# caishiqing/voice-tts

Measured on AMD Instinct MI355X. Metric: audio_seconds_per_second, higher is better.
Workload: dtype bf16

## Files before the change

include/ixtts_hip.h:

```cpp
#ifndef IXTTS_HIP_H
#define IXTTS_HIP_H

#include <stddef.h>
#include <stdint.h>

#ifdef __cplusplus
extern "C" {
#endif

#define IXTTS_OK 0
#define IXTTS_ERR_ARG (-1)
#define IXTTS_ERR_HIP (-2)
#define IXTTS_ERR_STATE (-3)
#define IXTTS_ERR_NOMEM (-4)
#define IXTTS_ERR_NAME (-5)

const char* ixtts_version(void);
const char* ixtts_last_error(void);

int ixtts_aa_snake_f32(const float* x_dev, float* y_dev, const float* up12_dev, const float* down12_dev,
                       const float* log_alpha_dev, const float* log_beta_dev, int B, int C, int T, void* stream);

size_t ixtts_attn_full_workspace_bytes(int B, int H, int T);
int ixtts_attn_full_f32(const float* q_dev, const float* k_dev, const float* v_dev, float* out_dev, int B, int H, int T,
// ... 144 lines not shown
int ixtts_gpt_decode(ixtts_gpt* h, int n_active, int n_steps, const ixtts_sampler_cfg* sc, void* stream);
int ixtts_gpt_decode_slots(ixtts_gpt* h, int n_active, int n_steps, const ixtts_sampler_cfg* per_slot, const uint32_t* rng_stream,
                           void* stream);
int ixtts_gpt_read(ixtts_gpt* h, int b, int32_t* ids_host, int cap, int* n_ids, int* finished, void* stream);
int ixtts_gpt_read_logits(ixtts_gpt* h, int b, float* logits_host, void* stream);
int ixtts_gpt_read_probs(ixtts_gpt* h, int b, float* probs_host, void* stream);
int ixtts_gpt_set_bans(ixtts_gpt* h, int slot, const int32_t* always_host, int n_always, const int32_t* first_host, int n_first,
                       void* stream);
int ixtts_gpt_set_sequence_bias(ixtts_gpt* h, int slot, const int32_t* ids_flat_host, const int32_t* lens_host, const float* biases_host,
                                int n, void* stream);
int ixtts_gpt_set_forced_eos(ixtts_gpt* h, int slot, const int32_t* ids_host, int n, void* stream);
int ixtts_gpt_force_next(ixtts_gpt* h, int b, int32_t token, void* stream);

int ixtts_gpt_beam_begin(ixtts_gpt* h, int num_beams, void* stream);
int ixtts_gpt_beam_decode(ixtts_gpt* h, int n_steps, const ixtts_sampler_cfg* sc, void* stream);
int ixtts_gpt_beam_read(ixtts_gpt* h, int max_new, int32_t* ids_host, int cap, int* n_ids, int* done, float* score,
                        float* beam_scores_host, int32_t* last_tokens_host, int32_t* beam_idx_host, void* stream);
int ixtts_gpt_beam_force(ixtts_gpt* h, const int32_t* picks_host, int n, void* stream);

int ixtts_gpt_beam_begin_group(ixtts_gpt* h, int group, int num_beams, uint64_t rng_stream, void* stream);
int ixtts_gpt_beam_park_group(ixtts_gpt* h, int group, void* stream);
int ixtts_gpt_beam_decode_groups(ixtts_gpt* h, int n_groups, int n_steps, const ixtts_sampler_cfg* sc, void* stream);
int ixtts_gpt_beam_decode_groups_cfg(ixtts_gpt* h, int n_groups, int n_steps, const ixtts_sampler_cfg* per_group, void* stream);
int ixtts_gpt_beam_read_group(ixtts_gpt* h, int group, int max_new, int32_t* ids_host, int cap, int* n_ids, int* done, float* score,
                              float* beam_scores_host, int32_t* last_tokens_host, int32_t* beam_idx_host, void* stream);
int ixtts_gpt_beam_force_group(ixtts_gpt* h, int group, const int32_t* picks_host, int n, void* stream);

int ixtts_gpt_latent(ixtts_gpt* h, const float* prefix_dev, int n_prefix, const int32_t* codes_dev, int n,
                     float* latent_dev, void* stream);
int ixtts_gpt_latent_many(ixtts_gpt* h, int n, const float* const* prefix_dev, const int* n_prefix, const int32_t* const* codes_dev,
                          const int* n_codes, float* const* latent_dev, int rows_max, void* stream);
int ixtts_gpt_latent_plan(const int* n_prefix, const int* n_codes, int n, int row_cap, int* pass_of);

int ixtts_gpt_bench_gemv(ixtts_gpt* h, int which, int layer, int batch, void* stream);
double ixtts_gpt_step_bytes(const ixtts_gpt* h, int B, int S);

int ixtts_gpt_max_batch(void);
int ixtts_gpt_max_batch_for(int weight_dtype);

int ixtts_gpt_destroy(ixtts_gpt* h);

#define IXTTS_QWEN_TOPK_MAX 64
#define IXTTS_QWEN_MAX_EOS 8
#define IXTTS_QWEN_MAX_SLOTS 4

typedef struct ixtts_qwen_cfg {
  int hidden_size;
  int layers;
  int heads;
  int kv_heads;
  int head_dim;
  int intermediate_size;
  int vocab_size;
  float rms_norm_eps;
  float rope_theta;
  int tie_word_embeddings;
  int max_seq;
  int weight_dtype;
  int n_eos;
  int eos_ids[IXTTS_QWEN_MAX_EOS];
} ixtts_qwen_cfg;

typedef struct ixtts_qwen_sampling {
  int do_sample;
  float temperature;
  int top_k;
// ... 60 lines not shown
```

voice-tts_amd/_lib.py:

```python
import ctypes as C
import os

HERE = os.path.dirname(os.path.abspath(__file__))
LIB_PATH = os.environ.get("IXTTS_LIB") or os.path.join(HERE, "libixtts_hip.so")

MAX_STAGES = 8
MAX_RESK = 4
BIGVGAN_TILE_SLOTS = 6


class BigVGANCfg(C.Structure):
    _fields_ = [
        ("num_mels", C.c_int), ("upsample_initial_channel", C.c_int), ("n_stages", C.c_int),
        ("upsample_rates", C.c_int * MAX_STAGES), ("upsample_kernel_sizes", C.c_int * MAX_STAGES),
        ("n_resblock_kernels", C.c_int), ("resblock_kernel_sizes", C.c_int * MAX_RESK),
        ("resblock_dilations", (C.c_int * 3) * MAX_RESK), ("max_frames", C.c_int), ("fast_sin", C.c_int),
    ]


class GptCfg(C.Structure):
    _fields_ = [
        ("model_dim", C.c_int), ("layers", C.c_int), ("heads", C.c_int), ("n_mel_codes", C.c_int),
        ("n_mel_pos", C.c_int), ("n_text_tokens", C.c_int), ("n_text_pos", C.c_int),
        ("start_mel_token", C.c_int), ("stop_mel_token", C.c_int), ("max_seq", C.c_int),
# ... 91 lines not shown
    "ixtts_bigvgan_forward_varlen": (C.c_int, [_P, _P, _P, _P, C.c_int, C.c_int, _P, _P]),
    "ixtts_bigvgan_tile_launches": (C.c_int, [_P, C.POINTER(C.c_int64), C.POINTER(C.c_int)]),
    "ixtts_bigvgan_flops": (C.c_double, [_P, C.c_int, C.c_int]),
    "ixtts_bigvgan_destroy": (C.c_int, [_P]),
    "ixtts_gpt_create": (C.c_int, [C.POINTER(_P), C.POINTER(GptCfg)]),
    "ixtts_gpt_set_tensor": (C.c_int, [_P, C.c_char_p, _P, C.POINTER(C.c_int64), C.c_int]),
    "ixtts_gpt_finalize": (C.c_int, [_P]),
    "ixtts_gpt_arena": (C.c_int, [_P, C.POINTER(_P), C.POINTER(C.c_size_t)]),
    "ixtts_gpt_adopt_arena": (C.c_int, [_P]),
    "ixtts_gpt_share_arena": (C.c_int, [_P, _P]),
    "ixtts_gpt_prefill": (C.c_int, [_P, C.c_int, _P, C.c_int, C.c_int, _P]),
    "ixtts_gpt_prefill_many": (C.c_int, [_P, C.c_int, C.POINTER(C.c_int), C.POINTER(_P), C.POINTER(C.c_int), C.POINTER(C.c_int), C.c_int, _P]),
    "ixtts_gpt_prefill_plan": (C.c_int, [C.POINTER(C.c_int), C.POINTER(C.c_int), C.c_int, C.c_int, C.POINTER(C.c_int)]),
    "ixtts_gpt_decode": (C.c_int, [_P, C.c_int, C.c_int, C.POINTER(SamplerCfg), _P]),
    "ixtts_gpt_decode_slots": (C.c_int, [_P, C.c_int, C.c_int, C.POINTER(SamplerCfg), C.POINTER(C.c_uint32), _P]),
    "ixtts_gpt_read": (C.c_int, [_P, C.c_int, _P, C.c_int, C.POINTER(C.c_int), C.POINTER(C.c_int), _P]),
    "ixtts_gpt_read_logits": (C.c_int, [_P, C.c_int, _P, _P]),
    "ixtts_gpt_beam_begin": (C.c_int, [_P, C.c_int, _P]),
    "ixtts_gpt_beam_decode": (C.c_int, [_P, C.c_int, C.POINTER(SamplerCfg), _P]),
    "ixtts_gpt_beam_read": (C.c_int, [_P, C.c_int, _P, C.c_int, C.POINTER(C.c_int), C.POINTER(C.c_int), C.POINTER(C.c_float), _P, _P, _P, _P]),
    "ixtts_gpt_beam_force": (C.c_int, [_P, _P, C.c_int, _P]),
    "ixtts_gpt_beam_begin_group": (C.c_int, [_P, C.c_int, C.c_int, C.c_uint64, _P]),
    "ixtts_gpt_beam_park_group": (C.c_int, [_P, C.c_int, _P]),
    "ixtts_gpt_beam_decode_groups": (C.c_int, [_P, C.c_int, C.c_int, C.POINTER(SamplerCfg), _P]),
    "ixtts_gpt_beam_decode_groups_cfg": (C.c_int, [_P, C.c_int, C.c_int, C.POINTER(SamplerCfg), _P]),
    "ixtts_gpt_beam_read_group":(C.c_int, [_P, C.c_int, C.c_int, _P, C.c_int, C.POINTER(C.c_int), C.POINTER(C.c_int), C.POINTER(C.c_float), _P, _P, _P, _P]),
    "ixtts_gpt_beam_force_group": (C.c_int, [_P, C.c_int, _P, C.c_int, _P]),
    "ixtts_gpt_read_probs": (C.c_int, [_P, C.c_int, _P, _P]),
    "ixtts_gpt_force_next": (C.c_int, [_P, C.c_int, C.c_int32, _P]),
    "ixtts_gpt_set_bans": (C.c_int, [_P, C.c_int, _P, C.c_int, _P, C.c_int, _P]),
    "ixtts_gpt_set_sequence_bias": (C.c_int, [_P, C.c_int, _P, _P, _P, C.c_int, _P]),
    "ixtts_gpt_set_forced_eos": (C.c_int, [_P, C.c_int, _P, C.c_int, _P]),
    "ixtts_gpt_latent": (C.c_int, [_P, _P, C.c_int, _P, C.c_int, _P, _P]),
    "ixtts_gpt_latent_many": (C.c_int, [_P, C.c_int, C.POINTER(_P), C.POINTER(C.c_int), C.POINTER(_P), C.POINTER(C.c_int), C.POINTER(_P), C.c_int, _P]),
    "ixtts_gpt_latent_plan": (C.c_int, [C.POINTER(C.c_int), C.POINTER(C.c_int), C.c_int, C.c_int, C.POINTER(C.c_int)]),
    "ixtts_gpt_bench_gemv": (C.c_int, [_P, C.c_int, C.c_int, C.c_int, _P]),
    "ixtts_gpt_step_bytes": (C.c_double, [_P, C.c_int, C.c_int]),
    "ixtts_gpt_max_batch": (C.c_int, []),
    "ixtts_gpt_max_batch_for": (C.c_int, [C.c_int]),
    "ixtts_gpt_destroy": (C.c_int, [_P]),
    "ixtts_qwen_create": (C.c_int, [C.POINTER(_P), C.POINTER(QwenCfg)]),
    "ixtts_qwen_set_tensor": (C.c_int, [_P, C.c_char_p, _P, C.POINTER(C.c_int64), C.c_int]),
    "ixtts_qwen_finalize": (C.c_int, [_P]),
    "ixtts_qwen_prefill": (C.c_int, [_P, _P, C.c_int, _P]),
    "ixtts_qwen_step": (C.c_int, [_P, C.c_int, C.POINTER(QwenSampling), _P]),
    "ixtts_qwen_read": (C.c_int, [_P, _P, C.c_int, C.POINTER(C.c_int), C.POINTER(C.c_int), _P]),
    "ixtts_qwen_generate": (C.c_int, [_P, C.c_int, C.POINTER(QwenSampling), _P, C.c_int, C.POINTER(C.c_int), C.POINTER(C.c_int), _P]),
    "ixtts_qwen_read_logits": (C.c_int, [_P, _P, _P]),
    "ixtts_qwen_read_kept": (C.c_int, [_P, _P, _P, C.c_int, C.POINTER(C.c_int), _P]),
    "ixtts_qwen_draw": (C.c_int, [_P, C.c_uint64, C.c_int, _P, _P]),
    "ixtts_qwen_step_bytes": (C.c_double, [_P, C.c_int]),
    "ixtts_qwen_create_slots": (C.c_int, [C.POINTER(_P), C.POINTER(QwenCfg), C.c_int]),
    "ixtts_qwen_prefill_slots": (C.c_int, [_P, C.c_int, _P, _P, _P]),
    "ixtts_qwen_step_slots": (C.c_int, [_P, C.c_int, C.c_int, C.POINTER(QwenSampling), _P]),
    "ixtts_qwen_generate_slots": (C.c_int, [_P, C.c_int, C.c_int, C.POINTER(QwenSampling), _P]),
    "ixtts_qwen_read_slot": (C.c_int, [_P, C.c_int, _P, C.c_int, C.POINTER(C.c_int), C.POINTER(C.c_int), _P]),
    "ixtts_qwen_read_logits_slot": (C.c_int, [_P, C.c_int, _P, _P]),
    "ixtts_qwen_read_kept_slot": (C.c_int, [_P, C.c_int, _P, _P, C.c_int, C.POINTER(C.c_int), _P]),
    "ixtts_qwen_destroy": (C.c_int, [_P]),
    "ixtts_resample_tile": (C.c_int, []),
    "ixtts_resample_varlen_f32": (C.c_int, [_P, C.c_long, _P, C.c_long, _P, C.c_int, C.c_long, _P, C.c_long, _P, C.c_int, C.c_int, C.c_int, C.c_int, _P]),
    "ixtts_pcm_assemble": (C.c_int, [_P, C.c_long, _P, C.c_long, _P, C.c_int, C.c_int, _P]),
    "ixtts_loudness_measure": (C.c_int, [_P, C.c_long, _P, C.c_int, _P, _P, C.c_int, C.c_long, _P, _P, C.c_long, _P]),
    "ixtts_loudness_gain": (C.c_int, [_P, _P, C.c_long, _P, _P, C.c_int, _P, _P, _P]),
    "ixtts_pcm_assemble_gain": (C.c_int, [_P, C.c_long, _P, C.c_long, _P, C.c_int, _P, C.c_int, C.c_int, _P]),
}
# ... 57 lines not shown
```

voice-tts_amd/csrc/gpt_engine.h:

```cpp
#pragma once
#include <map>
#include <string>
#include <vector>

#include "common.h"

namespace ixtts {

constexpr int MAXB = 32;
constexpr int MAXB_F32 = 16;
constexpr int MAXB_REG = 4;
constexpr int STEPS_PER_GRAPH = 8;
constexpr int BEAM_MAX = 4;
constexpr int MAXG = MAXB / 2;
constexpr int BEAM_LCP_STRIDE = BEAM_MAX * BEAM_MAX + BEAM_MAX;
constexpr int BEAM_FORCED_STRIDE = 2 * BEAM_MAX;

enum TKind { T_VEC = 0, T_MAT_T = 1, T_MAT_N = 2, T_EMB = 3 };

struct TDesc {
  size_t off = 0;
  int kind = T_VEC;
  int64_t d0 = 0, d1 = 0;
  size_t stage_off = 0;
// ... 57 lines not shown
  unsigned int rng_host[ixtts::MAXB] = {};
  float* scratch = nullptr;
  size_t scratch_floats = 0;
  hipStream_t cap_stream = nullptr;
  hipGraphExec_t step_exec[ixtts::MAXB + 1][ixtts::NBKT + 1] = {};
  hipGraphExec_t multi_exec[ixtts::MAXB + 1][ixtts::NBKT + 1] = {};
  bool mlp_fused = false;
  void* wprx = nullptr;
  float* mlp_part = nullptr;
  unsigned* mlp_ctr = nullptr;
  float* h2 = nullptr;
  float* hc = nullptr;
  bool wide = false;
  int pf_per = 2;
  bool attn_split = true;
  int attn_bucket = ixtts::NBKT;
  int host_prompt_len[ixtts::MAXB + 2];
  int host_gen_est[ixtts::MAXB + 2];
  int num_beams = 0;
  int beam_groups = 1;
  bool group_live[ixtts::MAXG] = {};
  bool group_begun[ixtts::MAXG] = {};
  unsigned long long* beam_stream = nullptr;
  float *beam_scores = nullptr, *hyp_score = nullptr, *hyp_worst = nullptr;
  int *beam_src = nullptr, *hyp_len = nullptr, *n_hyp = nullptr, *beam_done = nullptr, *beam_forced_flag = nullptr;
  int32_t *hyp_tok = nullptr, *beam_forced = nullptr;
  float* beam_cand_v = nullptr;
  int *beam_cand_i = nullptr, *beam_cand_n = nullptr;
  bool beam_every_row = false;
  int* beam_lcp = nullptr;
  hipGraphExec_t beam_exec[ixtts::MAXG + 1][ixtts::NBKT + 1] = {}, beam_multi_exec[ixtts::MAXG + 1][ixtts::NBKT + 1] = {};
  int beam_exec_nb = 0;
  float *rx = nullptr, *rxn = nullptr, *rq = nullptr, *ratt = nullptr, *rff = nullptr;
  std::vector<uint8_t> pf_host;
  uint8_t* pf_dev = nullptr;
  size_t pf_bytes = 0;
  std::vector<uint8_t> lm_host;
  uint8_t* lm_dev = nullptr;
  size_t lm_bytes = 0;
};

#define A_F32(off) reinterpret_cast<float*>(h->arena + (off))
#define A_PTR(off) reinterpret_cast<void*>(h->arena + (off))



namespace ixtts {
int forward_rows(ixtts_gpt* h, int slot, int T, int pos0, int valid_from, hipStream_t st);
}

namespace ixtts {
struct PackSeq {
  const float* embeds;
  int slot, T, pos0, row0;
};
struct PackedPass {
  const PackSeq* seqs;
  const int* tiles;
  const int* row_at;
  const int* row_seq;
  int n_seq, n_tiles, T;
  bool keys_rebased = false;
};
struct LatentSeq {
  const float* prefix;
  const int32_t* codes;
// ... 19 lines not shown
```

voice-tts_amd/csrc/gpt_engine.hip:

```cpp
#define IXTTS_ENGINE_TU 1
#include <type_traits>

#include "gpt_engine.h"
#include "gpt_kernels.h"
#include "gpt_wide.h"

using namespace ixtts;

#ifdef IXTTS_TRACE
static int g_trace_seq = 0;
#define IXTTS_TRACE_ARG , g_trace_seq++
#else
#define IXTTS_TRACE_ARG
#endif
template <typename WT, typename KVT, int K, int ROWS, int UNITS, int B, int INP, int EPI, int WPB = 4, bool XLDS = false>
static int launch_gemv(const GemvArgs& a, hipStream_t st) {
  auto kern = gemv_reg_kernel<WT, K, ROWS, UNITS, B, INP, EPI, KVT, WPB, XLDS>;
  const int n_units = (a.N + ROWS - 1) / ROWS;
  const int grid = ceil_div(n_units, WPB * UNITS);
  hipLaunchKernelGGL(kern, dim3(grid), dim3(64 * WPB), 0, st, a.wt, a.xin, a.bias, a.out, a.N, a.slot0, a.out_stride, a.smax, a.kcache, a.vcache,
                     a.cur_len, a.heads, a.nsplit, a.ln_w, a.ln_b, a.aux, a.xout IXTTS_PF_ARGS(a) IXTTS_TRACE_ARG);
  return IXTTS_OK;
}

// ... 1438 lines not shown
        if (pos + Ti > smax) {
          set_error("gpt_latent_many: entry %d would end at cache position %d of %d", i, pos + Ti, smax);
          return IXTTS_ERR_STATE;
        }
        const int q = tb.n_seq, row0 = tb.rows;
        tb.add(hb, nullptr, slot, Ti, pos, q, row0, h->H * smax);
        ls[q] = LatentSeq{prefix_dev[i], codes_dev[i], latent_dev[i], P, n_codes[i]};
        for (int t = P; t < Ti; ++t) mel_row[mel++] = row0 + t;
        pos += ceil_div(Ti, 64) * 64;
      }
      IX_HIP(hipMemcpyAsync(h->lm_dev, hb, tb.bytes, hipMemcpyHostToDevice, st));
      PackedPass pk = tb.pass(h->lm_dev, 0, n_seq, 0, n_tiles, 0, T);
      pk.keys_rebased = true;
      LatentPass lp;
      lp.lseqs = reinterpret_cast<const LatentSeq*>(h->lm_dev + tb.off_rec);
      lp.mel_row = reinterpret_cast<const int*>(h->lm_dev + tb.off_ints);
      lp.n_mel = n_mel;
      IX_TRY(pack_latent_rows(h, pk, lp, st));
      IX_TRY(forward_rows_packed(h, pk, st));
      IX_TRY(scatter_latent_rows(h, pk, lp, st));
    }
    i0 = i1;
  }
  IX_HIP(hipGetLastError());
  return IXTTS_OK;
}

extern "C" int ixtts_gpt_bench_gemv(ixtts_gpt* h, int which, int layer, int batch, void* stream) {
  NEED_READY(h, "gpt_bench_gemv");
  IX_ARG(layer >= 0 && layer < h->L && batch >= 1 && batch <= h->cfg.max_batch, "gpt_bench_gemv: bad argument");
  return do_gemv_which(h, which, layer, batch, (hipStream_t)stream);
}

extern "C" int ixtts_gpt_max_batch(void) { return MAXB_F32; }

extern "C" int ixtts_gpt_max_batch_for(int weight_dtype) {
  if (weight_dtype == IXTTS_DTYPE_BF16 || weight_dtype == IXTTS_DTYPE_F16) return MAXB;
  return weight_dtype == IXTTS_DTYPE_F32 ? MAXB_F32 : 0;
}

extern "C" double ixtts_gpt_step_bytes(const ixtts_gpt* h, int B, int S) {
  if (!h) return 0.0;
  const double D = h->D, FF = h->FF, V = h->V, L = h->L, es = (double)h->esize;
  double mat = L * (3 * D * D + D * D + 2 * D * FF) + V * D;
  double vec = L * (2 * D + 3 * D + D + 2 * D + FF + D) + 4 * D + V;
  double kv_read = (double)B * 2 * L * S * D * es;
  double kv_write = (double)B * 2 * L * D * es;
  double emb = (double)B * 2 * D * 4;
  return mat * es + vec * 4 + kv_read + kv_write + emb;
}

extern "C" int ixtts_gpt_destroy(ixtts_gpt* h) {
  if (!h) return IXTTS_OK;
  for (int k = 0; k <= NBKT; ++k) {
    for (int b = 0; b <= MAXB; ++b) {
      if (h->step_exec[b][k]) hipGraphExecDestroy(h->step_exec[b][k]);
      if (h->multi_exec[b][k]) hipGraphExecDestroy(h->multi_exec[b][k]);
    }
    for (int g = 0; g <= MAXG; ++g) {
      if (h->beam_exec[g][k]) hipGraphExecDestroy(h->beam_exec[g][k]);
      if (h->beam_multi_exec[g][k]) hipGraphExecDestroy(h->beam_multi_exec[g][k]);
    }
  }
  if (h->cap_stream) hipStreamDestroy(h->cap_stream);
  if (h->arena_borrowed) h->arena = nullptr;
  void* ptrs[] = {h->arena, h->stage, h->kc, h->vc, h->h, h->q, h->ff, h->att, h->part, h->logits, h->rowbuf, h->cur_len, h->gen_count,
// ... 31 lines not shown
```

voice-tts_amd/csrc/gpt_rows.hip:

```cpp
#include "gpt_engine.h"
#include "gpt_kernels.h"

namespace ixtts {

typedef float f32x16 __attribute__((ext_vector_type(16)));
typedef __bf16 bf16x8 __attribute__((ext_vector_type(8)));
typedef _Float16 f16x8 __attribute__((ext_vector_type(8)));

template <typename ET>
struct RowsEl;
template <>
struct RowsEl<bf16> {
  typedef bf16x8 vec8;
  __device__ static __forceinline__ f32x16 mfma(const vec8& a, const vec8& b, const f32x16& c) { return __builtin_amdgcn_mfma_f32_32x32x16_bf16(a, b, c, 0, 0, 0); }
};
template <>
struct RowsEl<f16> {
  typedef f16x8 vec8;
  __device__ static __forceinline__ f32x16 mfma(const vec8& a, const vec8& b, const f32x16& c) { return __builtin_amdgcn_mfma_f32_32x32x16_f16(a, b, c, 0, 0, 0); }
};

__device__ __forceinline__ unsigned int pack_bf16x2(float a, float b) {
  const unsigned short lo = __builtin_bit_cast(unsigned short, (__bf16)a);
  const unsigned short hi = __builtin_bit_cast(unsigned short, (__bf16)b);
// ... 232 lines not shown
          } else {
            const int which = n / g.D;
            const int c = n - which * g.D;
            const int hh = c / HD, d = c % HD;
            KVT* cache = reinterpret_cast<KVT*>(which == 1 ? g.kcache : g.vcache);
            store_kv(cache + ((size_t)hh * g.smax + g.pos0 + m) * HD + d, v);
          }
        }
      }
    }
}

struct GemmArgs16 {
  const unsigned short* A;
  const unsigned short* wt;
  const float* bias;
  void* out;
  void* kcache;
  void* vcache;
  int T, N, K, pos0, smax, D;
};

struct GemmArgs16Packed : GemmArgs16 {
  const int* row_at;
};

__device__ __forceinline__ void glds16(const void* gsrc, void* lds_wave_base) {
  __builtin_amdgcn_global_load_lds((const __attribute__((address_space(1))) void*)gsrc, (__attribute__((address_space(3))) void*)lds_wave_base, 16, 0, 0);
}

constexpr int G16_NBUF = 2;
constexpr int G16_TILE = 128 * 64 * 2;
constexpr int G16_SMEM = G16_NBUF * 2 * G16_TILE;

template <int EPI, typename KVT, typename GA = GemmArgs16>
__global__ __launch_bounds__(256) void gemm_rows_bf16_kernel(GA g) {
  using EL = RowsEl<KVT>;
  typedef typename EL::vec8 vec8;
  constexpr int BM = 128, BN = 128, BK = 64, TILE = G16_TILE, NBUF = G16_NBUF;
  extern __shared__ __attribute__((aligned(1024))) unsigned char smem_raw[];
  unsigned char (*smem)[2][TILE] = reinterpret_cast<unsigned char (*)[2][TILE]>(smem_raw);
  const int tid = threadIdx.x, lane = tid & 63, wave = tid >> 6;
  const int wm = wave >> 1, wn = wave & 1;
  const int l31 = lane & 31, lh = lane >> 5;
  const int m0 = blockIdx.y * BM, n0 = blockIdx.x * BN;

  f32x16 acc[2][2];
#pragma unroll
  for (int mi = 0; mi < 2; ++mi)
#pragma unroll
    for (int j = 0; j < 2; ++j)
#pragma unroll
      for (int r = 0; r < 16; ++r) acc[mi][j][r] = 0.f;

  const unsigned short* asrc[4];
  const unsigned short* wsrc[4];
#pragma unroll
  for (int i = 0; i < 4; ++i) {
    const int row = (wave * 4 + i) * 8 + (lane >> 3);
    const int gran = (lane & 7) ^ ((row >> 1) & 7);
    asrc[i] = g.A + (size_t)min(m0 + row, g.T - 1) * g.K + gran * 8;
    wsrc[i] = g.wt + (size_t)min(n0 + row, g.N - 1) * g.K + gran * 8;
  }
  auto issue = [&](int kt, int buf) {
#pragma unroll
    for (int i = 0; i < 4; ++i) {
      glds16(asrc[i] + kt * BK, &smem[buf][0][(wave * 4 + i) * 1024]);
      glds16(wsrc[i] + kt * BK, &smem[buf][1][(wave * 4 + i) * 1024]);
    }
  };
  const int nkt = g.K / BK;
#pragma unroll
  for (int p = 0; p < NBUF - 1; ++p) issue(min(p, nkt - 1), p);
  for (int kt = 0; kt < nkt; ++kt) {
    issue(min(kt + NBUF - 1, nkt - 1), (kt + NBUF - 1) % NBUF);
    static_assert(NBUF == 2, "the immediate below is 8 * (NBUF - 1)");
    asm volatile("s_waitcnt vmcnt(8)" ::: "memory");
    __builtin_amdgcn_s_barrier();
    const unsigned char* At = smem[kt % NBUF][0];
    const unsigned char* Wt = smem[kt % NBUF][1];
#pragma unroll
    for (int kk = 0; kk < BK / 16; ++kk) {
      vec8 a[2], b[2];
#pragma unroll
      for (int mi = 0; mi < 2; ++mi) {
        const int row = wm * 64 + mi * 32 + l31;
        a[mi] = *reinterpret_cast<const vec8*>(At + row * 128 + (((kk * 2 + lh) ^ ((row >> 1) & 7)) << 4));
      }
#pragma unroll
      for (int j = 0; j < 2; ++j) {
        const int row = wn * 64 + j * 32 + l31;
        b[j] = *reinterpret_cast<const vec8*>(Wt + row * 128 + (((kk * 2 + lh) ^ ((row >> 1) & 7)) << 4));
      }
#pragma unroll
      for (int mi = 0; mi < 2; ++mi)
#pragma unroll
        for (int j = 0; j < 2; ++j) acc[mi][j] = EL::mfma(a[mi], b[j], acc[mi][j]);
    }
    __builtin_amdgcn_s_barrier();
  }
  float bias[2];
  int ncol[2];
#pragma unroll
  for (int j = 0; j < 2; ++j) {
    ncol[j] = n0 + wn * 64 + j * 32 + l31;
    bias[j] = g.bias[min(ncol[j], g.N - 1)];
  }
  if constexpr (EPI == RE_RESID) {
    float* xo = reinterpret_cast<float*>(g.out);
    float old[2][2][16];
#pragma unroll
    for (int mi = 0; mi < 2; ++mi)
#pragma unroll
      for (int j = 0; j < 2; ++j)
#pragma unroll
        for (int r = 0; r < 16; ++r) {
          const int m = min(m0 + wm * 64 + mi * 32 + (r & 3) + 8 * (r >> 2) + 4 * lh, g.T - 1);
          old[mi][j][r] = xo[(size_t)m * g.N + min(ncol[j], g.N - 1)];
        }
#pragma unroll
    for (int mi = 0; mi < 2; ++mi)
#pragma unroll
      for (int j = 0; j < 2; ++j)
#pragma unroll
        for (int r = 0; r < 16; ++r) {
          const int m = m0 + wm * 64 + mi * 32 + (r & 3) + 8 * (r >> 2) + 4 * lh;
          if (m < g.T && ncol[j] < g.N) xo[(size_t)m * g.N + ncol[j]] = old[mi][j][r] + (acc[mi][j][r] + bias[j]);
        }
  } else if constexpr (EPI == RE_QKV_PACKED) {
    int at[2][16] = {};
    if (n0 + BN > g.D) {
#pragma unroll
      for (int mi = 0; mi < 2; ++mi)
#pragma unroll
        for (int r = 0; r < 16; ++r) at[mi][r] = g.row_at[min(m0 + wm * 64 + mi * 32 + (r & 3) + 8 * (r >> 2) + 4 * lh, g.T - 1)];
    }
#pragma unroll
    for (int mi = 0; mi < 2; ++mi)
#pragma unroll
      for (int j = 0; j < 2; ++j) {
        const int n = ncol[j];
#pragma unroll
        for (int r = 0; r < 16; ++r) {
          const int m = m0 + wm * 64 + mi * 32 + (r & 3) + 8 * (r >> 2) + 4 * lh;
          if (m >= g.T || n >= g.N) continue;
          const float v = acc[mi][j][r] + bias[j];
          if (n < g.D) {
            reinterpret_cast<float*>(g.out)[(size_t)m * g.D + n] = v;
          } else {
            const int which = n / g.D;
            const int c = n - which * g.D;
            const int hh = c / HD, d = c % HD;
            KVT* cache = reinterpret_cast<KVT*>(which == 1 ? g.kcache : g.vcache);
            store_kv(cache + ((size_t)hh * g.smax + at[mi][r]) * HD + d, v);
          }
        }
      }
  } else {
#pragma unroll
    for (int mi = 0; mi < 2; ++mi)
#pragma unroll
      for (int j = 0; j < 2; ++j) {
        const int n = ncol[j];
#pragma unroll
        for (int r = 0; r < 16; ++r) {
          const int m = m0 + wm * 64 + mi * 32 + (r & 3) + 8 * (r >> 2) + 4 * lh;
          if (m >= g.T || n >= g.N) continue;
          const float v = acc[mi][j][r] + bias[j];
          if constexpr (EPI == RE_GELU) {
            const float u2 = 1.5957691216057308f * (v + 0.044715f * v * v * v);
            store_kv(reinterpret_cast<KVT*>(g.out) + (size_t)m * g.N + n, v / (1.0f + __expf(-u2)));
          } else {
            if (n < g.D) {
              reinterpret_cast<float*>(g.out)[(size_t)m * g.D + n] = v;
            } else {
              const int which = n / g.D;
              const int c = n - which * g.D;
              const int hh = c / HD, d = c % HD;
              KVT* cache = reinterpret_cast<KVT*>(which == 1 ? g.kcache : g.vcache);
              store_kv(cache + ((size_t)hh * g.smax + g.pos0 + m) * HD + d, v);
            }
          }
        }
      }
  }
}

struct AttnRowsArgs {
  const float* q;
  const void* kcache;
  const void* vcache;
  void* out;
  int T, D, smax, pos0, valid_from;
};

template <typename KVT, typename OT = float>
__global__ __launch_bounds__(256) void attn_rows_kernel(AttnRowsArgs a) {
#define ROWS_ROW ((int)blockIdx.y)
#define ROWS_K0 0
// ... 89 lines not shown
__device__ __forceinline__ void attn_rows_flash_seq(const AttnRowsArgs& a, const int q0) {
#define FLASH_Q0 q0
#include "attn_rows_flash_body.h"
#undef FLASH_Q0
}
template <typename KVT, typename OT>
__global__ __launch_bounds__(256) void attn_rows_flash_packed_kernel(AttnPackedArgs p) {
  const int2 t = p.tiles[blockIdx.y];
  attn_rows_flash_seq<KVT, OT>(packed_seq_args<KVT, OT>(p, t.x), t.y);
}

static bool rows_attn_legacy() {
  static const bool legacy = getenv("IXTTS_ROWS_ATTN") && !strcmp(getenv("IXTTS_ROWS_ATTN"), "legacy");
  return legacy;
}

template <typename KVT, typename OT>
static void launch_attn_rows(ixtts_gpt* h, const AttnRowsArgs& a, hipStream_t st) {
  if (rows_attn_legacy()) hipLaunchKernelGGL((attn_rows_kernel<KVT, OT>), dim3(h->H, a.T), dim3(256), 0, st, a);
  else hipLaunchKernelGGL((attn_rows_flash_kernel<KVT, OT>), dim3(h->H, ceil_div(a.T, 128)), dim3(256), 0, st, a);
}

template <typename KVT, typename OT>
static void launch_attn_packed(ixtts_gpt* h, const PackedPass& pk, const void* kc_layer, const void* vc_layer, void* out, hipStream_t st) {
  const bool legacy = rows_attn_legacy();
  AttnPackedArgs p;
  p.q = h->rq; p.kcache = kc_layer; p.vcache = vc_layer; p.out = out; p.seqs = pk.seqs; p.tiles = reinterpret_cast<const int2*>(pk.tiles);
  p.row_seq = pk.row_seq; p.D = h->D; p.smax = h->smax; p.H = h->H;
  if (legacy && pk.keys_rebased) hipLaunchKernelGGL((attn_rows_packed_rebased_kernel<KVT, OT>), dim3(h->H, pk.T), dim3(256), 0, st, p);
  else if (legacy) hipLaunchKernelGGL((attn_rows_packed_kernel<KVT, OT>), dim3(h->H, pk.T), dim3(256), 0, st, p);
  else hipLaunchKernelGGL((attn_rows_flash_packed_kernel<KVT, OT>), dim3(h->H, pk.n_tiles), dim3(256), 0, st, p);
}

template <typename WT, typename KVT>
struct RowsPath {
  typedef GemmArgs16 Args;
  typedef GemmArgs16Packed ArgsPacked;
  typedef KVT Act;
  template <int EPI, typename GA>
  static int gemm(const GA& g, hipStream_t st) {
    static const hipError_t attr = hipFuncSetAttribute((const void*)gemm_rows_bf16_kernel<EPI, KVT, GA>, hipFuncAttributeMaxDynamicSharedMemorySize, G16_SMEM);
    IX_HIP(attr);
    hipLaunchKernelGGL((gemm_rows_bf16_kernel<EPI, KVT, GA>), dim3(ceil_div(g.N, 128), ceil_div(g.T, 128)), dim3(256), G16_SMEM, st, g);
    return IXTTS_OK;
  }
};
template <typename KVT>
struct RowsPath<float, KVT> {
  typedef GemmArgs Args;
  typedef GemmArgsPacked ArgsPacked;
  typedef float Act;
  template <int EPI, typename GA>
  static int gemm(const GA& g, hipStream_t st) {
    if (g.T >= 512) {
      hipLaunchKernelGGL((gemm_rows_kernel<float, EPI, KVT, 128, GA>), dim3(ceil_div(g.N, GBN), ceil_div(g.T, 128)), dim3(256), 0, st, g);
    } else {
      hipLaunchKernelGGL((gemm_rows_kernel<float, EPI, KVT, 64, GA>), dim3(ceil_div(g.N, GBN), ceil_div(g.T, 64)), dim3(256), 0, st, g);
    }
    return IXTTS_OK;
  }
};

template <typename WT, typename KVT, int D>
static int forward_rows_impl(ixtts_gpt* h, int slot, int T, int pos0, int valid_from, hipStream_t st, const PackedPass* pk) {
  using P = RowsPath<WT, KVT>;
  using Act = typename P::Act;
  const size_t lstride = (size_t)h->slots * D * h->smax * sizeof(KVT);
  const size_t sstride = (size_t)D * h->smax * sizeof(KVT);
  Act* xn = reinterpret_cast<Act*>(h->rxn);
  Act* att = reinterpret_cast<Act*>(h->ratt);
  Act* ff = reinterpret_cast<Act*>(h->rff);
  typename P::Args g;
  g.T = T; g.pos0 = pos0; g.smax = h->smax; g.D = D;
  auto operands = [&](const void* A, size_t w, size_t bias, void* out, int N, int K) {
    g.A = static_cast<decltype(g.A)>(A); g.wt = static_cast<decltype(g.wt)>(A_PTR(w)); g.bias = A_F32(bias);
    g.out = static_cast<decltype(g.out)>(out); g.N = N; g.K = K;
  };
  for (int l = 0; l < h->L; ++l) {
    const LayerOff& o = h->lo[l];
    uint8_t* kc = (uint8_t*)h->kc + l * lstride + slot * sstride;
    uint8_t* vc = (uint8_t*)h->vc + l * lstride + slot * sstride;
    hipLaunchKernelGGL((ln_rows_kernel<D, Act>), dim3(ceil_div(T, 4)), dim3(256), 0, st, h->rx, xn, T);
    operands(xn, o.wqkv, o.bqkv, h->rq, 3 * D, D);
    g.kcache = kc; g.vcache = vc;
    if (pk) {
      typename P::ArgsPacked gp;
      static_cast<typename P::Args&>(gp) = g;
      gp.row_at = pk->row_at;
      IX_TRY((P::template gemm<RE_QKV_PACKED>(gp, st)));
      launch_attn_packed<KVT, Act>(h, *pk, kc, vc, att, st);
    } else {
      IX_TRY((P::template gemm<RE_QKV>(g, st)));
      AttnRowsArgs a;
      a.q = h->rq; a.kcache = kc; a.vcache = vc; a.out = att; a.T = T; a.D = D; a.smax = h->smax; a.pos0 = pos0; a.valid_from = valid_from;
      launch_attn_rows<KVT, Act>(h, a, st);
    }
    operands(att, o.wo, o.bo, h->rx, D, D);
    IX_TRY((P::template gemm<RE_RESID>(g, st)));
    hipLaunchKernelGGL((ln_rows_kernel<D, Act>), dim3(ceil_div(T, 4)), dim3(256), 0, st, h->rx, xn, T);
    operands(xn, o.wfc, o.bfc, ff, 4 * D, D);
    IX_TRY((P::template gemm<RE_GELU>(g, st)));
    operands(ff, o.wpr, o.bpr, h->rx, D, 4 * D);
    IX_TRY((P::template gemm<RE_RESID>(g, st)));
  }
  IX_HIP(hipGetLastError());
  return IXTTS_OK;
}

static int forward_rows_any(ixtts_gpt* h, int slot, int T, int pos0, int valid_from, hipStream_t st, const PackedPass* pk) {
  if (T <= 0) return IXTTS_OK;
  const bool wide = h->D == 1280;
  switch (h->cfg.weight_dtype) {
    case IXTTS_DTYPE_F32:
      return wide ? forward_rows_impl<float, float, 1280>(h, slot, T, pos0, valid_from, st, pk) : forward_rows_impl<float, float, 128>(h, slot, T, pos0, valid_from, st, pk);
    case IXTTS_DTYPE_F16:
      return wide ? forward_rows_impl<f16, f16, 1280>(h, slot, T, pos0, valid_from, st, pk) : forward_rows_impl<f16, f16, 128>(h, slot, T, pos0, valid_from, st, pk);
    default:
      return wide ? forward_rows_impl<bf16, bf16, 1280>(h, slot, T, pos0, valid_from, st, pk) : forward_rows_impl<bf16, bf16, 128>(h, slot, T, pos0, valid_from, st, pk);
  }
}

int forward_rows(ixtts_gpt* h, int slot, int T, int pos0, int valid_from, hipStream_t st) { return forward_rows_any(h, slot, T, pos0, valid_from, st, nullptr); }

int forward_rows_packed(ixtts_gpt* h, const PackedPass& p, hipStream_t st) { return forward_rows_any(h, 0, p.T, 0, 0, st, &p); }

__global__ __launch_bounds__(256) void pack_rows_kernel(float* __restrict__ x, const PackSeq* __restrict__ seqs, const int* __restrict__ row_seq,
                                                         const float* __restrict__ start_emb, const float* __restrict__ mel_pos0, int D) {
  const int row = blockIdx.x;
  const PackSeq s = seqs[row_seq[row]];
  const int r = row - s.row0;
  float* dst = x + (size_t)row * D;
  if (r == s.T - 1) {
    for (int i = threadIdx.x; i < D; i += blockDim.x) dst[i] = start_emb[i] + mel_pos0[i];
  } else {
    const float* src = s.embeds + (size_t)(s.pos0 + r) * D;
    for (int i = threadIdx.x; i < D; i += blockDim.x) dst[i] = src[i];
// ... 100 lines not shown
```

voice-tts_amd/gpt_engine.py:

```python
import ctypes as C

import numpy as np
import torch

from . import _lib
from .weights import GPT_CFG

GPT_DTYPES = {"f32": 0, "bf16": 1, "f16": 2}


def _dtype_code(dtype):
    if dtype not in GPT_DTYPES:
        raise ValueError(f"GPT weight dtype {dtype!r}: expected one of " + ", ".join(GPT_DTYPES))
    return GPT_DTYPES[dtype]


def resolve_gpt_dtype(use_fp16, gpt_dtype=None, env=None):
    import os

    if gpt_dtype is None:
        gpt_dtype = (os.environ if env is None else env).get("IXTTS_GPT_DTYPE") or None
        if gpt_dtype is not None:
            gpt_dtype = gpt_dtype.strip().lower()
    if gpt_dtype is None:
# ... 163 lines not shown
                t = t.detach().to("cpu", torch.float32).contiguous()
                shape = (C.c_int64 * t.dim())(*t.shape)
                _lib.check(L.ixtts_gpt_set_tensor(self._h, name.encode(), t.data_ptr(), shape, t.dim()), f"ixtts_gpt_set_tensor({name})")
            _lib.check(L.ixtts_gpt_finalize(self._h), "ixtts_gpt_finalize")
        self._loaded = True
        return self

    def arena(self):
        p, n = C.c_void_p(), C.c_size_t()
        _lib.check(_lib.lib().ixtts_gpt_arena(self._h, C.byref(p), C.byref(n)), "ixtts_gpt_arena")
        return p.value, n.value

    def adopt_arena(self):
        _lib.check(_lib.lib().ixtts_gpt_adopt_arena(self._h), "ixtts_gpt_adopt_arena")
        self._loaded = True

    def share_arena(self, owner):
        with torch.cuda.device(self.device):
            _lib.check(_lib.lib().ixtts_gpt_share_arena(self._h, owner._h), "ixtts_gpt_share_arena")
        self._owner = owner
        self._loaded = True
        return self

    def _stream(self):
        return _lib.current_stream_ptr()

    def prefill(self, slot, embeds, n_left_pad=0):
        e = embeds.to(self.device, torch.float32).contiguous()
        assert e.dim() == 2 and e.shape[1] == self.D
        with torch.cuda.device(self.device):
            rc = _lib.lib().ixtts_gpt_prefill(self._h, slot, e.data_ptr(), e.shape[0], int(n_left_pad), self._stream())
        _lib.check(rc, "ixtts_gpt_prefill")
        self._keep = e

    def prefill_many(self, entries, rows_max=0):
        entries = list(entries)
        n = len(entries)
        keep = []
        for slot, embeds, n_left_pad in entries:
            e = embeds.to(self.device, torch.float32).contiguous()
            assert e.dim() == 2 and e.shape[1] == self.D
            keep.append(e)
        slots = (C.c_int * max(n, 1))(*[int(s) for s, _, _ in entries])
        ptrs = (C.c_void_p * max(n, 1))(*[e.data_ptr() for e in keep])
        rows = (C.c_int * max(n, 1))(*[int(e.shape[0]) for e in keep])
        pads = (C.c_int * max(n, 1))(*[int(p) for _, _, p in entries])
        with torch.cuda.device(self.device):
            rc = _lib.lib().ixtts_gpt_prefill_many(self._h, n, slots, ptrs, rows, pads, int(rows_max), self._stream())
        _lib.check(rc, "ixtts_gpt_prefill_many")
        if keep:
            self._keep_many = keep

    @staticmethod
    def prefill_plan(n_rows, n_left_pad, row_cap):
        n = len(n_rows)
        assert len(n_left_pad) == n
        out = (C.c_int * max(n, 1))()
        rc = _lib.lib().ixtts_gpt_prefill_plan((C.c_int * max(n, 1))(*map(int, n_rows)), (C.c_int * max(n, 1))(*map(int, n_left_pad)), n, int(row_cap), out)
        if rc < 0:
            _lib.check(rc, "ixtts_gpt_prefill_plan")
        return list(out[:n]), rc

    @staticmethod
    def _sampler_cfg(v):
        return _lib.SamplerCfg(v["repetition_penalty"], v["temperature"], int(v["top_k"]), v["top_p"], int(bool(v["do_sample"])),
                               int(bool(v["suppress_stop"])), int(v["seed"]), float(v["typical_mass"]), float(v.get("length_penalty", 0.0)),
# ... 317 lines not shown
```

Baseline: 42.03.

## Add pipelined 4-stage bf16 rows GEMM with occupancy-based tile selection

Adds a 4-stage ring-buffered variant of the bf16 rows GEMM that issues global-to-LDS copies three k-tiles ahead and interleaves LDS reads and copies with MFMAs using hand-placed asm and schedule barriers. Tile sizes of 64 or 128 in each dimension are chosen per launch: the smallest tile whose grid fits within the CU count (twice the count for 64x64). The aim is to hide memory latency and fill more CUs in prefill/latent GEMMs with small T. The cost is more LDS per block, more complex code and template instantiations, and a host-side launch counter, with an env override back to the old kernel.

```diff
diff --git a/include/ixtts_hip.h b/include/ixtts_hip.h
--- a/include/ixtts_hip.h
+++ b/include/ixtts_hip.h
@@ -200,6 +200,10 @@
                           const int* n_codes, float* const* latent_dev, int rows_max, void* stream);
 int ixtts_gpt_latent_plan(const int* n_prefix, const int* n_codes, int n, int row_cap, int* pass_of);
 
+int ixtts_gpt_rows_gemm_mode(ixtts_gpt* h, int mode);
+#define IXTTS_GPT_ROWS_GEMM_SLOTS 5
+int ixtts_gpt_rows_gemm_launches(const ixtts_gpt* h, int64_t* counts );
+
 int ixtts_gpt_bench_gemv(ixtts_gpt* h, int which, int layer, int batch, void* stream);
 double ixtts_gpt_step_bytes(const ixtts_gpt* h, int B, int S);
 
diff --git a/voice-tts_amd/_lib.py b/voice-tts_amd/_lib.py
--- a/voice-tts_amd/_lib.py
+++ b/voice-tts_amd/_lib.py
@@ -147,6 +147,8 @@
     "ixtts_gpt_set_sequence_bias": (C.c_int, [_P, C.c_int, _P, _P, _P, C.c_int, _P]),
     "ixtts_gpt_set_forced_eos": (C.c_int, [_P, C.c_int, _P, C.c_int, _P]),
     "ixtts_gpt_latent": (C.c_int, [_P, _P, C.c_int, _P, C.c_int, _P, _P]),
+    "ixtts_gpt_rows_gemm_mode": (C.c_int, [_P, C.c_int]),
+    "ixtts_gpt_rows_gemm_launches": (C.c_int, [_P, C.POINTER(C.c_int64)]),
     "ixtts_gpt_latent_many": (C.c_int, [_P, C.c_int, C.POINTER(_P), C.POINTER(C.c_int), C.POINTER(_P), C.POINTER(C.c_int), C.POINTER(_P), C.c_int, _P]),
     "ixtts_gpt_latent_plan": (C.c_int, [C.POINTER(C.c_int), C.POINTER(C.c_int), C.c_int, C.c_int, C.POINTER(C.c_int)]),
     "ixtts_gpt_bench_gemv": (C.c_int, [_P, C.c_int, C.c_int, C.c_int, _P]),
diff --git a/voice-tts_amd/csrc/gpt_engine.h b/voice-tts_amd/csrc/gpt_engine.h
--- a/voice-tts_amd/csrc/gpt_engine.h
+++ b/voice-tts_amd/csrc/gpt_engine.h
@@ -113,6 +113,8 @@
   hipGraphExec_t beam_exec[ixtts::MAXG + 1][ixtts::NBKT + 1] = {}, beam_multi_exec[ixtts::MAXG + 1][ixtts::NBKT + 1] = {};
   int beam_exec_nb = 0;
   float *rx = nullptr, *rxn = nullptr, *rq = nullptr, *ratt = nullptr, *rff = nullptr;
+  int rows_gemm_mode = 0;
+  long long rows_gemm_launches[IXTTS_GPT_ROWS_GEMM_SLOTS] = {};
   std::vector<uint8_t> pf_host;
   uint8_t* pf_dev = nullptr;
   size_t pf_bytes = 0;
diff --git a/voice-tts_amd/csrc/gpt_engine.hip b/voice-tts_amd/csrc/gpt_engine.hip
--- a/voice-tts_amd/csrc/gpt_engine.hip
+++ b/voice-tts_amd/csrc/gpt_engine.hip
@@ -1494,6 +1494,19 @@
   return do_gemv_which(h, which, layer, batch, (hipStream_t)stream);
 }
 
+extern "C" int ixtts_gpt_rows_gemm_mode(ixtts_gpt* h, int mode) {
+  IX_ARG(h, "gpt_rows_gemm_mode: null handle");
+  IX_ARG(mode >= 0 && mode <= IXTTS_GPT_ROWS_GEMM_SLOTS, "gpt_rows_gemm_mode: mode %d is none of 0 (auto), 1 (parent), 2..5 (pipelined tiles)", mode);
+  h->rows_gemm_mode = mode;
+  return IXTTS_OK;
+}
+
+extern "C" int ixtts_gpt_rows_gemm_launches(const ixtts_gpt* h, int64_t* counts) {
+  IX_ARG(h && counts, "gpt_rows_gemm_launches: null argument");
+  for (int i = 0; i < IXTTS_GPT_ROWS_GEMM_SLOTS; ++i) counts[i] = h->rows_gemm_launches[i];
+  return IXTTS_OK;
+}
+
 extern "C" int ixtts_gpt_max_batch(void) { return MAXB_F32; }
 
 extern "C" int ixtts_gpt_max_batch_for(int weight_dtype) {
diff --git a/voice-tts_amd/csrc/gpt_rows.hip b/voice-tts_amd/csrc/gpt_rows.hip
--- a/voice-tts_amd/csrc/gpt_rows.hip
+++ b/voice-tts_amd/csrc/gpt_rows.hip
@@ -288,27 +288,141 @@
 constexpr int G16_NBUF = 2;
 constexpr int G16_TILE = 128 * 64 * 2;
 constexpr int G16_SMEM = G16_NBUF * 2 * G16_TILE;
-
-template <int EPI, typename KVT, typename GA = GemmArgs16>
+constexpr int G16P_NST = 4, G16P_LEAD = 3;
+constexpr int g16p_smem(int BM, int BN) { return G16P_NST * (BM + BN) * 128; }
+
+typedef unsigned int u32x4 __attribute__((ext_vector_type(4)));
+
+template <int EPI, typename KVT, typename GA = GemmArgs16, int BM = 128, int BN = 128, int PIPE = 0>
 __global__ __launch_bounds__(256) void gemm_rows_bf16_kernel(GA g) {
   using EL = RowsEl<KVT>;
   typedef typename EL::vec8 vec8;
-  constexpr int BM = 128, BN = 128, BK = 64, TILE = G16_TILE, NBUF = G16_NBUF;
+  constexpr int BK = 64, MI = BM / 64, NJ = BN / 64;
+  static_assert((BM == 64 || BM == 128) && (BN == 64 || BN == 128), "tiles of 64 | 128 rows and columns");
+  static_assert(PIPE != 0 || (BM == 128 && BN == 128), "the two-buffer loop is built for 128 x 128");
   extern __shared__ __attribute__((aligned(1024))) unsigned char smem_raw[];
-  unsigned char (*smem)[2][TILE] = reinterpret_cast<unsigned char (*)[2][TILE]>(smem_raw);
   const int tid = threadIdx.x, lane = tid & 63, wave = tid >> 6;
   const int wm = wave >> 1, wn = wave & 1;
   const int l31 = lane & 31, lh = lane >> 5;
   const int m0 = blockIdx.y * BM, n0 = blockIdx.x * BN;
 
-  f32x16 acc[2][2];
-#pragma unroll
-  for (int mi = 0; mi < 2; ++mi)
-#pragma unroll
-    for (int j = 0; j < 2; ++j)
+  f32x16 acc[MI][NJ];
+#pragma unroll
+  for (int mi = 0; mi < MI; ++mi)
+#pragma unroll
+    for (int j = 0; j < NJ; ++j)
 #pragma unroll
       for (int r = 0; r < 16; ++r) acc[mi][j][r] = 0.f;
 
+  const int nkt = g.K / BK;
+  if constexpr (PIPE != 0) {
+    constexpr int NST = G16P_NST, LEAD = G16P_LEAD, STAGE = (BM + BN) * 128;
+    constexpr int NPA = BM / 32, NPW = BN / 32, NP = NPA + NPW;
+    constexpr int NM = 4 * MI * NJ;
+    static_assert(NST == 4 && LEAD == NST - 1, "(a), (b): copies 3 k-tiles ahead in a ring of 4");
+    static_assert(LEAD % NST != 0 && LEAD % NST != 1, "(b): the copy target is neither the stage of k-tile kt nor of kt + 1");
+    static_assert(NP <= NM, "every copy behind an MFMA of its own");
+    const int wv = __builtin_amdgcn_readfirstlane(wave);
+    const unsigned short* src[NP];
+    int dst[NP];
+#pragma unroll
+    for (int i = 0; i < NP; ++i) {
+      const bool isA = i < NPA;
+      const int piece = isA ? wv * NPA + i : wv * NPW + (i - NPA);
+      const int row = piece * 8 + (lane >> 3);
+      const int gran = (lane & 7) ^ ((row >> 1) & 7);
+      src[i] = isA ? g.A + (size_t)min(m0 + row, g.T - 1) * g.K + gran * 8
+                   : g.wt + (size_t)min(n0 + row, g.N - 1) * g.K + gran * 8;
+      dst[i] = (isA ? 0 : BM * 128) + piece * 1024;
+    }
+    auto issue_piece = [&](int kt, int i) { glds16(src[i] + kt * BK, smem_raw + (kt & (NST - 1)) * STAGE + dst[i]); };
+    const unsigned lds0 = (unsigned)(uintptr_t)(const __attribute__((address_space(3))) void*)smem_raw;
+    unsigned a_rel[4], w_rel[4];
+#pragma unroll
+    for (int kk = 0; kk < 4; ++kk) {
+      const int sw = ((kk * 2 + lh) ^ ((l31 >> 1) & 7)) << 4;
+      a_rel[kk] = lds0 + (unsigned)((wm * (BM / 2) + l31) * 128 + sw);
+      w_rel[kk] = lds0 + (unsigned)(BM * 128 + (wn * (BN / 2) + l31) * 128 + sw);
+    }
+    u32x4 fa[2][MI], fb[2][NJ];
+    auto read_issue = [&](u32x4 (&a)[MI], u32x4 (&b)[NJ], int stage, int kk) {
+      const unsigned aaddr = a_rel[kk] + (unsigned)(stage * STAGE), waddr = w_rel[kk] + (unsigned)(stage * STAGE);
+      if constexpr (MI == 2 && NJ == 2)
+        asm volatile("ds_read_b128 %0, %4\n ds_read_b128 %1, %4 offset:4096\n ds_read_b128 %2, %5\n ds_read_b128 %3, %5 offset:4096"
+                     : "=&v"(a[0]), "=&v"(a[1]), "=&v"(b[0]), "=&v"(b[1]) : "v"(aaddr), "v"(waddr) : "memory");
+      else if constexpr (MI == 2)
+        asm volatile("ds_read_b128 %0, %3\n ds_read_b128 %1, %3 offset:4096\n ds_read_b128 %2, %4"
+                     : "=&v"(a[0]), "=&v"(a[1]), "=&v"(b[0]) : "v"(aaddr), "v"(waddr) : "memory");
+      else if constexpr (NJ == 2)
+        asm volatile("ds_read_b128 %0, %3\n ds_read_b128 %1, %4\n ds_read_b128 %2, %4 offset:4096"
+                     : "=&v"(a[0]), "=&v"(b[0]), "=&v"(b[1]) : "v"(aaddr), "v"(waddr) : "memory");
+      else
+        asm volatile("ds_read_b128 %0, %2\n ds_read_b128 %1, %3" : "=&v"(a[0]), "=&v"(b[0]) : "v"(aaddr), "v"(waddr) : "memory");
+    };
+    auto read_wait = [&](u32x4 (&a)[MI], u32x4 (&b)[NJ]) {
+      if constexpr (MI == 2 && NJ == 2) asm volatile("s_waitcnt lgkmcnt(0)" : "+v"(a[0]), "+v"(a[1]), "+v"(b[0]), "+v"(b[1]) : : "memory");
+      else if constexpr (MI == 2) asm volatile("s_waitcnt lgkmcnt(0)" : "+v"(a[0]), "+v"(a[1]), "+v"(b[0]) : : "memory");
+      else if constexpr (NJ == 2) asm volatile("s_waitcnt lgkmcnt(0)" : "+v"(a[0]), "+v"(b[0]), "+v"(b[1]) : : "memory");
+      else asm volatile("s_waitcnt lgkmcnt(0)" : "+v"(a[0]), "+v"(b[0]) : : "memory");
+    };
+    auto ktile = [&](auto copy, auto next, auto sync, int kt) {
+      constexpr bool COPY = decltype(copy)::value, NEXT = decltype(next)::value, SYNC = decltype(sync)::value;
+      static_assert(NEXT || !COPY, "copies are only issued for k-tiles that will be read");
+      static_assert(NEXT || !SYNC, "the closing wait and barrier publish data to a later read block");
+      const int st = kt & (NST - 1), st_next = (kt + 1) & (NST - 1);
+#pragma unroll
+      for (int kk = 0; kk < 4; ++kk) {
+        const int c = kk & 1;
+        const bool READ = kk < 3 || NEXT;
+#pragma unroll
+        for (int mi = 0; mi < MI; ++mi)
+#pragma unroll
+          for (int j = 0; j < NJ; ++j) {
+            acc[mi][j] = EL::mfma(__builtin_bit_cast(vec8, fa[c][mi]), __builtin_bit_cast(vec8, fb[c][j]), acc[mi][j]);
+            const int m = kk * MI * NJ + mi * NJ + j;
+            if (READ && mi == 0 && j == 0) {
+              __builtin_amdgcn_sched_barrier(0);
+              read_issue(fa[1 - c], fb[1 - c], kk < 3 ? st : st_next, (kk + 1) & 3);
+              __builtin_amdgcn_sched_barrier(0);
+            }
+            if constexpr (COPY) {
+#pragma unroll
+              for (int q = 0; q < NP; ++q)
+                if (((2 * q + 1) * NM) / (2 * NP) == m) {
+                  __builtin_amdgcn_sched_barrier(0);
+                  issue_piece(kt + LEAD, q);
+                  __builtin_amdgcn_sched_barrier(0);
+                }
+            }
+          }
+        if (READ) read_wait(fa[1 - c], fb[1 - c]);
+      }
+      if constexpr (SYNC) {
+        if constexpr (COPY) asm volatile("s_waitcnt vmcnt(%0)" ::"n"(NP) : "memory");
+        else asm volatile("s_waitcnt vmcnt(0)" ::: "memory");
+        __builtin_amdgcn_s_barrier();
+        asm volatile("" ::: "memory");
+      }
+    };
+    constexpr std::true_type Y;
+    constexpr std::false_type N_;
+    for (int t = 0; t < LEAD && t < nkt; ++t)
+#pragma unroll
+      for (int q = 0; q < NP; ++q) issue_piece(t, q);
+    if (nkt >= LEAD) asm volatile("s_waitcnt vmcnt(%0)" ::"n"(NP) : "memory");
+    else asm volatile("s_waitcnt vmcnt(0)" ::: "memory");
+    __builtin_amdgcn_s_barrier();
+    asm volatile("" ::: "memory");
+    read_issue(fa[0], fb[0], 0, 0);
+    read_wait(fa[0], fb[0]);
+    int kt = 0;
+    for (; kt + LEAD < nkt; ++kt) ktile(Y, Y, Y, kt);
+    if (nkt >= 3) ktile(N_, Y, Y, kt++);
+    if (nkt >= 2) ktile(N_, Y, N_, kt++);
+    ktile(N_, N_, N_, kt);
+  } else {
+  constexpr int TILE = G16_TILE, NBUF = G16_NBUF;
+  unsigned char (*smem)[2][TILE] = reinterpret_cast<unsigned char (*)[2][TILE]>(smem_raw);
   const unsigned short* asrc[4];
   const unsigned short* wsrc[4];
 #pragma unroll
@@ -325,7 +439,6 @@
       glds16(wsrc[i] + kt * BK, &smem[buf][1][(wave * 4 + i) * 1024]);
     }
   };
-  const int nkt = g.K / BK;
 #pragma unroll
   for (int p = 0; p < NBUF - 1; ++p) issue(min(p, nkt - 1), p);
   for (int kt = 0; kt < nkt; ++kt) {
@@ -355,50 +468,51 @@
     }
     __builtin_amdgcn_s_barrier();
   }
-  float bias[2];
-  int ncol[2];
-#pragma unroll
-  for (int j = 0; j < 2; ++j) {
-    ncol[j] = n0 + wn * 64 + j * 32 + l31;
+  }
+  float bias[NJ];
+  int ncol[NJ];
+#pragma unroll
+  for (int j = 0; j < NJ; ++j) {
+    ncol[j] = n0 + wn * (BN / 2) + j * 32 + l31;
     bias[j] = g.bias[min(ncol[j], g.N - 1)];
   }
   if constexpr (EPI == RE_RESID) {
     float* xo = reinterpret_cast<float*>(g.out);
-    float old[2][2][16];
-#pragma unroll
-    for (int mi = 0; mi < 2; ++mi)
-#pragma unroll
-      for (int j = 0; j < 2; ++j)
+    float old[MI][NJ][16];
+#pragma unroll
+    for (int mi = 0; mi < MI; ++mi)
+#pragma unroll
+      for (int j = 0; j < NJ; ++j)
 #pragma unroll
         for (int r = 0; r < 16; ++r) {
-          const int m = min(m0 + wm * 64 + mi * 32 + (r & 3) + 8 * (r >> 2) + 4 * lh, g.T - 1);
+          const int m = min(m0 + wm * (BM / 2) + mi * 32 + (r & 3) + 8 * (r >> 2) + 4 * lh, g.T - 1);
           old[mi][j][r] = xo[(size_t)m * g.N + min(ncol[j], g.N - 1)];
         }
 #pragma unroll
-    for (int mi = 0; mi < 2; ++mi)
-#pragma unroll
-      for (int j = 0; j < 2; ++j)
+    for (int mi = 0; mi < MI; ++mi)
+#pragma unroll
+      for (int j = 0; j < NJ; ++j)
 #pragma unroll
         for (int r = 0; r < 16; ++r) {
-          const int m = m0 + wm * 64 + mi * 32 + (r & 3) + 8 * (r >> 2) + 4 * lh;
+          const int m = m0 + wm * (BM / 2) + mi * 32 + (r & 3) + 8 * (r >> 2) + 4 * lh;
           if (m < g.T && ncol[j] < g.N) xo[(size_t)m * g.N + ncol[j]] = old[mi][j][r] + (acc[mi][j][r] + bias[j]);
         }
   } else if constexpr (EPI == RE_QKV_PACKED) {
-    int at[2][16] = {};
+    int at[MI][16] = {};
     if (n0 + BN > g.D) {
 #pragma unroll
-      for (int mi = 0; mi < 2; ++mi)
-#pragma unroll
-        for (int r = 0; r < 16; ++r) at[mi][r] = g.row_at[min(m0 + wm * 64 + mi * 32 + (r & 3) + 8 * (r >> 2) + 4 * lh, g.T - 1)];
-    }
-#pragma unroll
-    for (int mi = 0; mi < 2; ++mi)
-#pragma unroll
-      for (int j = 0; j < 2; ++j) {
+      for (int mi = 0; mi < MI; ++mi)
+#pragma unroll
+        for (int r = 0; r < 16; ++r) at[mi][r] = g.row_at[min(m0 + wm * (BM / 2) + mi * 32 + (r & 3) + 8 * (r >> 2) + 4 * lh, g.T - 1)];
+    }
+#pragma unroll
+    for (int mi = 0; mi < MI; ++mi)
+#pragma unroll
+      for (int j = 0; j < NJ; ++j) {
         const int n = ncol[j];
 #pragma unroll
         for (int r = 0; r < 16; ++r) {
-          const int m = m0 + wm * 64 + mi * 32 + (r & 3) + 8 * (r >> 2) + 4 * lh;
+          const int m = m0 + wm * (BM / 2) + mi * 32 + (r & 3) + 8 * (r >> 2) + 4 * lh;
           if (m >= g.T || n >= g.N) continue;
           const float v = acc[mi][j][r] + bias[j];
           if (n < g.D) {
@@ -414,13 +528,13 @@
       }
   } else {
 #pragma unroll
-    for (int mi = 0; mi < 2; ++mi)
-#pragma unroll
-      for (int j = 0; j < 2; ++j) {
+    for (int mi = 0; mi < MI; ++mi)
+#pragma unroll
+      for (int j = 0; j < NJ; ++j) {
         const int n = ncol[j];
 #pragma unroll
         for (int r = 0; r < 16; ++r) {
-          const int m = m0 + wm * 64 + mi * 32 + (r & 3) + 8 * (r >> 2) + 4 * lh;
+          const int m = m0 + wm * (BM / 2) + mi * 32 + (r & 3) + 8 * (r >> 2) + 4 * lh;
           if (m >= g.T || n >= g.N) continue;
           const float v = acc[mi][j][r] + bias[j];
           if constexpr (EPI == RE_GELU) {
@@ -576,17 +690,49 @@
   else hipLaunchKernelGGL((attn_rows_flash_packed_kernel<KVT, OT>), dim3(h->H, pk.n_tiles), dim3(256), 0, st, p);
 }
 
+static long rows_cu_count() {
+  static const long n = [] {
+    int dev = 0, cus = 0;
+    return (hipGetDevice(&dev) == hipSuccess && hipDeviceGetAttribute(&cus, hipDeviceAttributeMultiprocessorCount, dev) == hipSuccess) ? (long)cus : 0L;
+  }();
+  return n;
+}
+static bool rows_gemm_parent() {
+  static const bool parent = getenv("IXTTS_ROWS_GEMM") && !strcmp(getenv("IXTTS_ROWS_GEMM"), "parent");
+  return parent;
+}
+static int rows_gemm_variant(const ixtts_gpt* h, int T, int N) {
+  if (h->rows_gemm_mode > 0) return h->rows_gemm_mode - 1;
+  if (rows_gemm_parent()) return 0;
+  static const int bm[4] = {64, 64, 128, 128}, bn[4] = {64, 128, 64, 128};
+  for (int v = 0; v < 4; ++v)
+    if ((long)ceil_div(T, bm[v]) * ceil_div(N, bn[v]) <= (v == 0 ? 2 : 1) * rows_cu_count()) return v + 1;
+  return 0;
+}
 template <typename WT, typename KVT>
 struct RowsPath {
   typedef GemmArgs16 Args;
   typedef GemmArgs16Packed ArgsPacked;
   typedef KVT Act;
+  template <int EPI, typename GA, int BM, int BN, int PIPE>
+  static int launch(const GA& g, hipStream_t st) {
+    constexpr int smem = PIPE ? g16p_smem(BM, BN) : G16_SMEM;
+    static const hipError_t attr = hipFuncSetAttribute((const void*)gemm_rows_bf16_kernel<EPI, KVT, GA, BM, BN, PIPE>, hipFuncAttributeMaxDynamicSharedMemorySize, smem);
+    IX_HIP(attr);
+    hipLaunchKernelGGL((gemm_rows_bf16_kernel<EPI, KVT, GA, BM, BN, PIPE>), dim3(ceil_div(g.N, BN), ceil_div(g.T, BM)), dim3(256), smem, st, g);
+    return IXTTS_OK;
+  }
   template <int EPI, typename GA>
-  static int gemm(const GA& g, hipStream_t st) {
-    static const hipError_t attr = hipFuncSetAttribute((const void*)gemm_rows_bf16_kernel<EPI, KVT, GA>, hipFuncAttributeMaxDynamicSharedMemorySize, G16_SMEM);
-    IX_HIP(attr);
-    hipLaunchKernelGGL((gemm_rows_bf16_kernel<EPI, KVT, GA>), dim3(ceil_div(g.N, 128), ceil_div(g.T, 128)), dim3(256), G16_SMEM, st, g);
-    return IXTTS_OK;
+  static int gemm(ixtts_gpt* h, const GA& g, hipStream_t st) {
+    const int v = rows_gemm_variant(h, g.T, g.N);
+    ++h->rows_gemm_launches[v];
+    switch (v) {
+      case 1: return launch<EPI, GA, 64, 64, 1>(g, st);
+      case 2: return launch<EPI, GA, 64, 128, 1>(g, st);
+      case 3: return launch<EPI, GA, 128, 64, 1>(g, st);
+      case 4: return launch<EPI, GA, 128, 128, 1>(g, st);
+    }
+    return launch<EPI, GA, 128, 128, 0>(g, st);
   }
 };
 template <typename KVT>
@@ -595,7 +741,7 @@
   typedef GemmArgsPacked ArgsPacked;
   typedef float Act;
   template <int EPI, typename GA>
-  static int gemm(const GA& g, hipStream_t st) {
+  static int gemm(ixtts_gpt*, const GA& g, hipStream_t st) {
     if (g.T >= 512) {
       hipLaunchKernelGGL((gemm_rows_kernel<float, EPI, KVT, 128, GA>), dim3(ceil_div(g.N, GBN), ceil_div(g.T, 128)), dim3(256), 0, st, g);
     } else {
@@ -631,21 +777,21 @@
       typename P::ArgsPacked gp;
       static_cast<typename P::Args&>(gp) = g;
       gp.row_at = pk->row_at;
-      IX_TRY((P::template gemm<RE_QKV_PACKED>(gp, st)));
+      IX_TRY((P::template gemm<RE_QKV_PACKED>(h, gp, st)));
       launch_attn_packed<KVT, Act>(h, *pk, kc, vc, att, st);
     } else {
-      IX_TRY((P::template gemm<RE_QKV>(g, st)));
+      IX_TRY((P::template gemm<RE_QKV>(h, g, st)));
       AttnRowsArgs a;
       a.q = h->rq; a.kcache = kc; a.vcache = vc; a.out = att; a.T = T; a.D = D; a.smax = h->smax; a.pos0 = pos0; a.valid_from = valid_from;
       launch_attn_rows<KVT, Act>(h, a, st);
     }
     operands(att, o.wo, o.bo, h->rx, D, D);
-    IX_TRY((P::template gemm<RE_RESID>(g, st)));
+    IX_TRY((P::template gemm<RE_RESID>(h, g, st)));
     hipLaunchKernelGGL((ln_rows_kernel<D, Act>), dim3(ceil_div(T, 4)), dim3(256), 0, st, h->rx, xn, T);
     operands(xn, o.wfc, o.bfc, ff, 4 * D, D);
-    IX_TRY((P::template gemm<RE_GELU>(g, st)));
+    IX_TRY((P::template gemm<RE_GELU>(h, g, st)));
     operands(ff, o.wpr, o.bpr, h->rx, D, 4 * D);
-    IX_TRY((P::template gemm<RE_RESID>(g, st)));
+    IX_TRY((P::template gemm<RE_RESID>(h, g, st)));
   }
   IX_HIP(hipGetLastError());
   return IXTTS_OK;
diff --git a/voice-tts_amd/gpt_engine.py b/voice-tts_amd/gpt_engine.py
--- a/voice-tts_amd/gpt_engine.py
+++ b/voice-tts_amd/gpt_engine.py
@@ -219,6 +219,16 @@
             rc = _lib.lib().ixtts_gpt_prefill(self._h, slot, e.data_ptr(), e.shape[0], int(n_left_pad), self._stream())
         _lib.check(rc, "ixtts_gpt_prefill")
         self._keep = e
+
+    ROWS_GEMM_VARIANTS = ("parent", "64x64", "64x128", "128x64", "128x128")
+
+    def rows_gemm_mode(self, mode):
+        _lib.check(_lib.lib().ixtts_gpt_rows_gemm_mode(self._h, int(mode)), "ixtts_gpt_rows_gemm_mode")
+
+    def rows_gemm_launches(self):
+        counts = (C.c_int64 * len(self.ROWS_GEMM_VARIANTS))()
+        _lib.check(_lib.lib().ixtts_gpt_rows_gemm_launches(self._h, counts), "ixtts_gpt_rows_gemm_launches")
+        return dict(zip(self.ROWS_GEMM_VARIANTS, (int(c) for c in counts)))
 
     def prefill_many(self, entries, rows_max=0):
         entries = list(entries)
```

After: 42.18 (median of 6 runs). No clear change (+0.3%).
